# igormq/aes-lac-2018

Hardware: AMD Instinct MI355X
Metric: train frames/sec, DeepSpeech2 5xBiGRU-800 (higher is better)
Workload: dtype f32

## Files before the change

### aes-lac-2018_amd/csrc/bn.hip

```cpp
#include "ds2_common.h"

namespace {

constexpr int NPART = 64;

template <int MODE>
__global__ __launch_bounds__(256) void bn2d_reduce_kernel(const float* __restrict__ x, const float* __restrict__ dy,
                                                          const float* __restrict__ mean_invstd,
                                                          const float* __restrict__ gamma,
                                                          const float* __restrict__ beta, int B, int C, int inner,
                                                          double* __restrict__ part) {
    const int c = blockIdx.y, p = blockIdx.x, tid = threadIdx.x;
    const int chunks = (inner + 1023) / 1024;
    const int items = B * chunks;
    float mu = 0.f, is = 0.f, ga = 0.f, be = 0.f;
    if (MODE == 1) {
        mu = mean_invstd[c];
        is = mean_invstd[C + c];
        ga = gamma[c];
        be = beta[c];
    }
    float s0 = 0.f, s1 = 0.f;
    for (int it = p; it < items; it += NPART) {
        const int b = it / chunks, ch = it % chunks;
        const size_t base = ((size_t)b * C + c) * inner;
        const int i0 = ch * 1024;
#pragma unroll
        for (int u = 0; u < 4; ++u) {
            const int i = i0 + u * 256 + tid;
            if (i < inner) {
                const float v = x[base + i];
                if (MODE == 0) {
                    s0 += v;
                    s1 += v * v;
                } else {
                    const float xh = (v - mu) * is;
                    const float y = ga * xh + be;
                    const float g = (y > 0.f && y < 20.f) ? dy[base + i] : 0.f;
                    s0 += g;
                    s1 += g * xh;
                }
            }
        }
    }
    double d0 = wave_sum_d((double)s0), d1 = wave_sum_d((double)s1);
    __shared__ double sm[4][2];
    if ((tid & 63) == 0) {
        sm[tid >> 6][0] = d0;
        sm[tid >> 6][1] = d1;
    }
    __syncthreads();
    if (tid == 0) {
        part[((size_t)c * NPART + p) * 2 + 0] = sm[0][0] + sm[1][0] + sm[2][0] + sm[3][0];
        part[((size_t)c * NPART + p) * 2 + 1] = sm[0][1] + sm[1][1] + sm[2][1] + sm[3][1];
    }
}

template <int MODE>
__global__ __launch_bounds__(256) void bn2d_reduce_vec_kernel(const float* __restrict__ x, const float* __restrict__ dy,
                                                              const float* __restrict__ mean_invstd,
                                                              const float* __restrict__ gamma,
                                                              const float* __restrict__ beta, int B, int C, int inner,
                                                              double* __restrict__ part) {
    const int c = blockIdx.y, p = blockIdx.x, tid = threadIdx.x;
    const int chunks = (inner + 1023) / 1024;
    const int items = B * chunks;
    float mu = 0.f, is = 0.f, ga = 0.f, be = 0.f;
    if (MODE == 1) {
        mu = mean_invstd[c];
        is = mean_invstd[C + c];
        ga = gamma[c];
        be = beta[c];
    }
    float s0 = 0.f, s1 = 0.f;
    auto take = [&](float v, float g) {
        if (MODE == 0) {
            s0 += v;
            s1 += v * v;
        } else {
            const float xh = (v - mu) * is;
            const float y = ga * xh + be;
            const float gm = (y > 0.f && y < 20.f) ? g : 0.f;
            s0 += gm;
            s1 += gm * xh;
        }
    };
    for (int it = p; it < items; it += NPART) {
        const int b = it / chunks, ch = it % chunks;
        const size_t base = ((size_t)b * C + c) * inner;
        const int h = min((int)((4 - (base & 3)) & 3), inner);
        const int nq = (inner - h) >> 2;
        const int q = ch * 256 + tid;
        if (q < nq) {
            const f32x4 v = *reinterpret_cast<const f32x4*>(x + base + h + 4 * (size_t)q);
            f32x4 g = {0.f, 0.f, 0.f, 0.f};
            if (MODE == 1) g = *reinterpret_cast<const f32x4*>(dy + base + h + 4 * (size_t)q);
#pragma unroll
            for (int e = 0; e < 4; ++e) take(v[e], g[e]);
        }
        if (ch == 0) {
            const int tail0 = h + 4 * nq, e = tid < 4 ? tid : tail0 + tid - 4;
            if ((tid < h) || (tid >= 4 && tid < 8 && e < inner)) take(x[base + e], MODE == 1 ? dy[base + e] : 0.f);
        }
    }
    double d0 = wave_sum_d((double)s0), d1 = wave_sum_d((double)s1);
    __shared__ double sm[4][2];
    if ((tid & 63) == 0) {
        sm[tid >> 6][0] = d0;
        sm[tid >> 6][1] = d1;
    }
    __syncthreads();
    if (tid == 0) {
        part[((size_t)c * NPART + p) * 2 + 0] = sm[0][0] + sm[1][0] + sm[2][0] + sm[3][0];
        part[((size_t)c * NPART + p) * 2 + 1] = sm[0][1] + sm[1][1] + sm[2][1] + sm[3][1];
    }
}

template <int MODE>
__global__ __launch_bounds__(256) void bn1d_reduce_kernel(const float* __restrict__ xa, const float* __restrict__ xb,
                                                          const float* __restrict__ dy,
                                                          const float* __restrict__ mean_invstd, int rows, int F,
                                                          double* __restrict__ part) {
    const int p = blockIdx.x, tid = threadIdx.x;
    const int col = blockIdx.y * 64 + (tid & 63), ry = tid >> 6;
    float mu = 0.f, is = 0.f;
    if (MODE == 1 && col < F) {
        mu = mean_invstd[col];
        is = mean_invstd[F + col];
    }
    float s0 = 0.f, s1 = 0.f;
    if (col < F) {
        for (int r = p * 4 + ry; r < rows; r += NPART * 4) {
            const size_t o = (size_t)r * F + col;
            float v = xa[o];
            if (xb) v += xb[o];
            if (MODE == 0) {
                s0 += v;
                s1 += v * v;
            } else {
                const float g = dy[o];
                s0 += g;
                s1 += g * (v - mu) * is;
            }
        }
    }
    __shared__ float sm[4][64][2];
    sm[ry][tid & 63][0] = s0;
    sm[ry][tid & 63][1] = s1;
    __syncthreads();
    if (ry == 0 && col < F) {
        const int l = tid & 63;
        const double d0 = (double)sm[0][l][0] + (double)sm[1][l][0] + (double)sm[2][l][0] + (double)sm[3][l][0];
        const double d1 = (double)sm[0][l][1] + (double)sm[1][l][1] + (double)sm[2][l][1] + (double)sm[3][l][1];
        part[((size_t)col * NPART + p) * 2 + 0] = d0;
        part[((size_t)col * NPART + p) * 2 + 1] = d1;
    }
}

__global__ __launch_bounds__(64) void bn_finalize_stats_kernel(const double* __restrict__ part, int C, double count,
                                                               float eps, float momentum, int use_running,
                                                               float* __restrict__ running_mean,
                                                               float* __restrict__ running_var,
                                                               float* __restrict__ mean_invstd) {
    const int c = blockIdx.x, lane = threadIdx.x;
    if (use_running) {
        if (lane == 0) {
            mean_invstd[c] = running_mean[c];
            mean_invstd[C + c] = (float)(1.0 / sqrt((double)running_var[c] + (double)eps));
        }
        return;
    }
    double s0 = part[((size_t)c * NPART + lane) * 2 + 0];
    double s1 = part[((size_t)c * NPART + lane) * 2 + 1];
    s0 = wave_sum_d(s0);
    s1 = wave_sum_d(s1);
    if (lane == 0) {
        const double mean = s0 / count;
        double var = s1 / count - mean * mean;
        if (var < 0.0) var = 0.0;
        mean_invstd[c] = (float)mean;
        mean_invstd[C + c] = (float)(1.0 / sqrt(var + (double)eps));
        if (running_mean) {
            const double unb = count > 1.0 ? var * count / (count - 1.0) : var;
            running_mean[c] = (float)((1.0 - momentum) * running_mean[c] + momentum * mean);
            running_var[c] = (float)((1.0 - momentum) * running_var[c] + momentum * unb);
        }
    }
}

__global__ __launch_bounds__(64) void bn_finalize_bwd_kernel(const double* __restrict__ part, int C, double count,
                                                             float* __restrict__ dgamma, float* __restrict__ dbeta,
                                                             float* __restrict__ coef) {
    const int c = blockIdx.x, lane = threadIdx.x;
    double s0 = part[((size_t)c * NPART + lane) * 2 + 0];
    double s1 = part[((size_t)c * NPART + lane) * 2 + 1];
    s0 = wave_sum_d(s0);
    s1 = wave_sum_d(s1);
    if (lane == 0) {
        dbeta[c] = (float)s0;
        dgamma[c] = (float)s1;
        coef[c] = (float)(s0 / count);
        coef[C + c] = (float)(s1 / count);
    }
}

__global__ __launch_bounds__(256) void bn2d_apply_kernel(const float* __restrict__ x,
                                                         const float* __restrict__ mean_invstd,
                                                         const float* __restrict__ gamma,
                                                         const float* __restrict__ beta, int C, int inner,
                                                         float* __restrict__ y) {
    const int bc = blockIdx.y, c = bc % C;
    const float sc = gamma[c] * mean_invstd[C + c];
    const float sh = beta[c] - mean_invstd[c] * sc;
    const size_t base = (size_t)bc * inner;
    for (int i = blockIdx.x * 256 + threadIdx.x; i < inner; i += gridDim.x * 256) {
        const float v = x[base + i] * sc + sh;
        y[base + i] = fminf(fmaxf(v, 0.f), 20.f);
    }
}

__global__ __launch_bounds__(256) void bn2d_apply_tbf_kernel(const float* __restrict__ x,
                                                             const float* __restrict__ mean_invstd,
                                                             const float* __restrict__ gamma,
                                                             const float* __restrict__ beta, int B, int C, int D,
                                                             int T, float* __restrict__ y) {
    __shared__ float tile[32][33];
    const int b = blockIdx.z;
    const int CD = C * D;
    const int t0 = blockIdx.x * 32, f0 = blockIdx.y * 32;
    const int tx = threadIdx.x & 31, ty = threadIdx.x >> 5;
#pragma unroll
    for (int i = 0; i < 32; i += 8) {
        const int f = f0 + ty + i, t = t0 + tx;
        if (f < CD && t < T) {
            const int c = f / D;
            const float sc = gamma[c] * mean_invstd[C + c];
            const float sh = beta[c] - mean_invstd[c] * sc;
            const float v = x[((size_t)b * CD + f) * T + t] * sc + sh;
            tile[ty + i][tx] = fminf(fmaxf(v, 0.f), 20.f);
        }
    }
    __syncthreads();
#pragma unroll
    for (int i = 0; i < 32; i += 8) {
        const int t = t0 + ty + i, f = f0 + tx;
        if (f < CD && t < T) y[((size_t)t * B + b) * CD + f] = tile[tx][ty + i];
    }
}

__global__ __launch_bounds__(256) void bn2d_bwd_apply_kernel(const float* __restrict__ x, const float* __restrict__ dy,
                                                             const float* __restrict__ mean_invstd,
                                                             const float* __restrict__ gamma,
                                                             const float* __restrict__ beta,
                                                             const float* __restrict__ coef, int C, int inner,
                                                             float* __restrict__ dx) {
    const int bc = blockIdx.y, c = bc % C;
    const float mu = mean_invstd[c], is = mean_invstd[C + c], ga = gamma[c], be = beta[c];
    const float mg = coef[c], mgx = coef[C + c];
    const size_t base = (size_t)bc * inner;
    for (int i = blockIdx.x * 256 + threadIdx.x; i < inner; i += gridDim.x * 256) {
        const float xh = (x[base + i] - mu) * is;
        const float yv = ga * xh + be;
        const float g = (yv > 0.f && yv < 20.f) ? dy[base + i] : 0.f;
        dx[base + i] = ga * is * (g - mg - xh * mgx);
    }
}

template <typename F>
__device__ __forceinline__ void bn2d_row_vec(size_t base, int inner, F&& f4, int bx, int nbx, int tid) {
    const int h = min((int)((4 - (base & 3)) & 3), inner);
    const int nq = (inner - h) >> 2;
    for (int q = bx * 256 + tid; q < nq; q += nbx * 256) f4(base + h + 4 * (size_t)q, 4);
    if (bx == 0) {
        const int tail0 = h + 4 * nq, e = tid < 4 ? tid : tail0 + tid - 4;
        if ((tid < h) || (tid >= 4 && tid < 8 && e < inner)) f4(base + e, 1);
    }
}

__global__ __launch_bounds__(256) void bn2d_bwd_apply_vec_kernel(const float* __restrict__ x, const float* __restrict__ dy,
                                                                 const float* __restrict__ mean_invstd,
                                                                 const float* __restrict__ gamma,
                                                                 const float* __restrict__ beta,
                                                                 const float* __restrict__ coef, int C, int inner,
                                                                 float* __restrict__ dx) {
    const int bc = blockIdx.y, c = bc % C;
    const float mu = mean_invstd[c], is = mean_invstd[C + c], ga = gamma[c], be = beta[c];
    const float mg = coef[c], mgx = coef[C + c];
    auto one = [&](float xv, float g) {
        const float xh = (xv - mu) * is;
        const float yv = ga * xh + be;
        const float gm = (yv > 0.f && yv < 20.f) ? g : 0.f;
        return ga * is * (gm - mg - xh * mgx);
    };
    bn2d_row_vec((size_t)bc * inner, inner, [&](size_t o, int n) {
        if (n == 4) {
            const f32x4 xv = *reinterpret_cast<const f32x4*>(x + o), g = *reinterpret_cast<const f32x4*>(dy + o);
            f32x4 r;
#pragma unroll
            for (int e = 0; e < 4; ++e) r[e] = one(xv[e], g[e]);
            *reinterpret_cast<f32x4*>(dx + o) = r;
        } else {
            dx[o] = one(x[o], dy[o]);
        }
    }, blockIdx.x, gridDim.x, threadIdx.x);
}

__global__ __launch_bounds__(256) void bn2d_apply_vec_kernel(const float* __restrict__ x,
                                                             const float* __restrict__ mean_invstd,
                                                             const float* __restrict__ gamma,
                                                             const float* __restrict__ beta, int C, int inner,
                                                             float* __restrict__ y) {
    const int bc = blockIdx.y, c = bc % C;
    const float sc = gamma[c] * mean_invstd[C + c];
    const float sh = beta[c] - mean_invstd[c] * sc;
    bn2d_row_vec((size_t)bc * inner, inner, [&](size_t o, int n) {
        if (n == 4) {
            const f32x4 xv = *reinterpret_cast<const f32x4*>(x + o);
            f32x4 r;
#pragma unroll
            for (int e = 0; e < 4; ++e) r[e] = fminf(fmaxf(xv[e] * sc + sh, 0.f), 20.f);
            *reinterpret_cast<f32x4*>(y + o) = r;
        } else {
            y[o] = fminf(fmaxf(x[o] * sc + sh, 0.f), 20.f);
        }
    }, blockIdx.x, gridDim.x, threadIdx.x);
}

__global__ __launch_bounds__(256) void bn1d_apply_kernel(const float* __restrict__ xa, const float* __restrict__ xb,
                                                         const float* __restrict__ mean_invstd,
                                                         const float* __restrict__ gamma,
                                                         const float* __restrict__ beta, size_t n, int F,
                                                         float* __restrict__ y) {
    const size_t stride = (size_t)gridDim.x * 256;
    for (size_t i = (size_t)blockIdx.x * 256 + threadIdx.x; i < n; i += stride) {
        const int col = (int)(i % F);
        float v = xa[i];
        if (xb) v += xb[i];
        const float sc = gamma[col] * mean_invstd[F + col];
        y[i] = (v - mean_invstd[col]) * sc + beta[col];
    }
}

__global__ __launch_bounds__(256) void bn1d_bwd_apply_kernel(const float* __restrict__ xa, const float* __restrict__ xb,
                                                             const float* __restrict__ dy,
                                                             const float* __restrict__ mean_invstd,
                                                             const float* __restrict__ gamma,
                                                             const float* __restrict__ coef, size_t n, int F,
                                                             float* __restrict__ dx) {
    const size_t stride = (size_t)gridDim.x * 256;
    for (size_t i = (size_t)blockIdx.x * 256 + threadIdx.x; i < n; i += stride) {
        const int col = (int)(i % F);
        float v = xa[i];
        if (xb) v += xb[i];
        const float is = mean_invstd[F + col];
        const float xh = (v - mean_invstd[col]) * is;
        dx[i] = gamma[col] * is * (dy[i] - coef[col] - xh * coef[F + col]);
    }
}

template <int MODE>
__global__ __launch_bounds__(256) void bn1d_reduce_vec_kernel(const f32x4* __restrict__ xa, const f32x4* __restrict__ xb,
                                                              const f32x4* __restrict__ dy,
                                                              const float* __restrict__ mean_invstd, int rows, int F,
                                                              double* __restrict__ part) {
    const int p = blockIdx.x, tid = threadIdx.x;
    const int F4 = F >> 2;
    const int cq = blockIdx.y * 64 + (tid & 63), ry = tid >> 6;
    f32x4 mu = {0.f, 0.f, 0.f, 0.f}, is = mu;
    if (MODE == 1 && cq < F4) {
        mu = *reinterpret_cast<const f32x4*>(mean_invstd + 4 * cq);
        is = *reinterpret_cast<const f32x4*>(mean_invstd + F + 4 * cq);
    }
    f32x4 s0 = {0.f, 0.f, 0.f, 0.f}, s1 = s0;
    if (cq < F4) {
        for (int r = p * 4 + ry; r < rows; r += NPART * 4) {
            const size_t o = (size_t)r * F4 + cq;
            f32x4 v = xa[o];
            if (xb) v += xb[o];
            if (MODE == 0) {
                s0 += v;
                s1 += v * v;
            } else {
                const f32x4 g = dy[o];
                s0 += g;
                s1 += g * (v - mu) * is;
            }
        }
    }
    __shared__ f32x4 sm[4][64][2];
    sm[ry][tid & 63][0] = s0;
    sm[ry][tid & 63][1] = s1;
    __syncthreads();
    if (ry == 0 && cq < F4) {
        const int l = tid & 63;
#pragma unroll
        for (int e = 0; e < 4; ++e) {
            const double d0 = (double)sm[0][l][0][e] + (double)sm[1][l][0][e] + (double)sm[2][l][0][e] + (double)sm[3][l][0][e];
            const double d1 = (double)sm[0][l][1][e] + (double)sm[1][l][1][e] + (double)sm[2][l][1][e] + (double)sm[3][l][1][e];
            part[((size_t)(4 * cq + e) * NPART + p) * 2 + 0] = d0;
            part[((size_t)(4 * cq + e) * NPART + p) * 2 + 1] = d1;
        }
    }
}

__global__ __launch_bounds__(256) void bn1d_apply_vec_kernel(const f32x4* __restrict__ xa, const f32x4* __restrict__ xb,
                                                             const float* __restrict__ mean_invstd,
                                                             const float* __restrict__ gamma,
                                                             const float* __restrict__ beta, size_t n4, int F4,
                                                             f32x4* __restrict__ y) {
    const size_t stride = (size_t)gridDim.x * 256;
    for (size_t i = (size_t)blockIdx.x * 256 + threadIdx.x; i < n4; i += stride) {
        const int c = 4 * (int)(i % F4);
        f32x4 v = xa[i];
        if (xb) v += xb[i];
        const f32x4 sc = *reinterpret_cast<const f32x4*>(gamma + c) * *reinterpret_cast<const f32x4*>(mean_invstd + 4 * F4 + c);
        y[i] = (v - *reinterpret_cast<const f32x4*>(mean_invstd + c)) * sc + *reinterpret_cast<const f32x4*>(beta + c);
    }
}

__global__ __launch_bounds__(256) void bn1d_bwd_apply_vec_kernel(const f32x4* __restrict__ xa, const f32x4* __restrict__ xb,
                                                                 const f32x4* __restrict__ dy,
                                                                 const float* __restrict__ mean_invstd,
                                                                 const float* __restrict__ gamma,
                                                                 const float* __restrict__ coef, size_t n4, int F4,
                                                                 f32x4* __restrict__ dx) {
    const size_t stride = (size_t)gridDim.x * 256;
    const int F = 4 * F4;
    for (size_t i = (size_t)blockIdx.x * 256 + threadIdx.x; i < n4; i += stride) {
        const int c = 4 * (int)(i % F4);
        f32x4 v = xa[i];
        if (xb) v += xb[i];
        const f32x4 is = *reinterpret_cast<const f32x4*>(mean_invstd + F + c);
        const f32x4 xh = (v - *reinterpret_cast<const f32x4*>(mean_invstd + c)) * is;
        dx[i] = *reinterpret_cast<const f32x4*>(gamma + c) * is *
                (dy[i] - *reinterpret_cast<const f32x4*>(coef + c) - xh * *reinterpret_cast<const f32x4*>(coef + F + c));
    }
}

inline bool aligned16(const void* p) { return ((uintptr_t)p & 15) == 0; }
inline bool vec4_ok(int F, const void* a, const void* b, const void* c, const void* d) {
    return (F & 3) == 0 && ((((uintptr_t)a) | ((uintptr_t)b) | ((uintptr_t)c) | ((uintptr_t)d)) & 15) == 0;
}

inline int ew_blocks(size_t n) {
    size_t b = (n + 255) / 256;
    if (b > 4096) b = 4096;
    if (b < 1) b = 1;
    return (int)b;
}

}

extern "C" size_t ds2_bn_ws_bytes(int C) { return (size_t)C * NPART * 2 * sizeof(double) + (size_t)C * 2 * sizeof(float); }

extern "C" int ds2_bn2d_stats(const float* x, int B, int C, int inner, float eps, float momentum, int use_running,
                              float* running_mean, float* running_var, float* mean_invstd, void* ws, void* stream) {
    DS2_CHECK_ARG(x && mean_invstd && ws && B > 0 && C > 0 && inner > 0);
    DS2_CHECK_ARG(!use_running || (running_mean && running_var));
    DS2_CHECK_ARG((running_mean == nullptr) == (running_var == nullptr));
    DS2_CHECK_ARG(C <= 65535);
    hipStream_t st = (hipStream_t)stream;
    double* part = (double*)ws;
    if (!use_running) {
        if (aligned16(x))
            hipLaunchKernelGGL((bn2d_reduce_vec_kernel<0>), dim3(NPART, C), dim3(256), 0, st, x, nullptr, nullptr, nullptr,
                               nullptr, B, C, inner, part);
        else
            hipLaunchKernelGGL((bn2d_reduce_kernel<0>), dim3(NPART, C), dim3(256), 0, st, x, nullptr, nullptr, nullptr,
                               nullptr, B, C, inner, part);
    }
    hipLaunchKernelGGL(bn_finalize_stats_kernel, dim3(C), dim3(64), 0, st, part, C, (double)B * inner, eps, momentum,
                       use_running, running_mean, running_var, mean_invstd);
    DS2_CHECK_LAUNCH();
    return DS2_OK;
}

extern "C" int ds2_bn2d_apply_htanh(const float* x, const float* mean_invstd, const float* gamma, const float* beta,
                                    int B, int C, int D, int T, int layout_tbf, float* y, void* stream) {
    DS2_CHECK_ARG(x && mean_invstd && gamma && beta && y && B > 0 && C > 0 && D > 0 && T > 0);
    hipStream_t st = (hipStream_t)stream;
    if (layout_tbf) {
        DS2_CHECK_ARG(B <= 65535);
        dim3 grid(ds2_cdiv(T, 32), ds2_cdiv(C * D, 32), B);
        hipLaunchKernelGGL(bn2d_apply_tbf_kernel, grid, dim3(256), 0, st, x, mean_invstd, gamma, beta, B, C, D, T, y);
    } else {
        DS2_CHECK_ARG((long long)B * C <= 65535);
        const int inner = D * T;
        if (aligned16(x) && aligned16(y)) {
            dim3 grid(min(ds2_cdiv(inner, 1024), 64), B * C);
            hipLaunchKernelGGL(bn2d_apply_vec_kernel, grid, dim3(256), 0, st, x, mean_invstd, gamma, beta, C, inner, y);
        } else {
            dim3 grid(min(ds2_cdiv(inner, 256), 64), B * C);
            hipLaunchKernelGGL(bn2d_apply_kernel, grid, dim3(256), 0, st, x, mean_invstd, gamma, beta, C, inner, y);
        }
    }
    DS2_CHECK_LAUNCH();
    return DS2_OK;
}

extern "C" int ds2_bn2d_htanh_bwd(const float* x, const float* dy, const float* mean_invstd, const float* gamma,
                                  const float* beta, int B, int C, int D, int T, float* dx, float* dgamma,
                                  float* dbeta, void* ws, void* stream) {
    DS2_CHECK_ARG(x && dy && mean_invstd && gamma && beta && dx && dgamma && dbeta && ws);
    DS2_CHECK_ARG(B > 0 && C > 0 && D > 0 && T > 0);
    DS2_CHECK_ARG((long long)B * C <= 65535);
    hipStream_t st = (hipStream_t)stream;
    const int inner = D * T;
    double* part = (double*)ws;
    float* coef = (float*)(part + (size_t)C * NPART * 2);
    const bool vec = aligned16(x) && aligned16(dy) && aligned16(dx);
    if (vec)
        hipLaunchKernelGGL((bn2d_reduce_vec_kernel<1>), dim3(NPART, C), dim3(256), 0, st, x, dy, mean_invstd, gamma, beta,
                           B, C, inner, part);
    else
        hipLaunchKernelGGL((bn2d_reduce_kernel<1>), dim3(NPART, C), dim3(256), 0, st, x, dy, mean_invstd, gamma, beta, B,
                           C, inner, part);
    hipLaunchKernelGGL(bn_finalize_bwd_kernel, dim3(C), dim3(64), 0, st, part, C, (double)B * inner, dgamma, dbeta,
                       coef);
    if (vec) {
        dim3 grid(min(ds2_cdiv(inner, 1024), 64), B * C);
        hipLaunchKernelGGL(bn2d_bwd_apply_vec_kernel, grid, dim3(256), 0, st, x, dy, mean_invstd, gamma, beta, coef, C,
                           inner, dx);
    } else {
        dim3 grid(min(ds2_cdiv(inner, 256), 64), B * C);
        hipLaunchKernelGGL(bn2d_bwd_apply_kernel, grid, dim3(256), 0, st, x, dy, mean_invstd, gamma, beta, coef, C, inner,
                           dx);
    }
    DS2_CHECK_LAUNCH();
    return DS2_OK;
}

extern "C" int ds2_bn1d_stats(const float* xa, const float* xb, int rows, int F, float eps, float momentum,
                              int use_running, float* running_mean, float* running_var, float* mean_invstd, void* ws,
                              void* stream) {
    DS2_CHECK_ARG(xa && mean_invstd && ws && rows > 0 && F > 0);
    DS2_CHECK_ARG(!use_running || (running_mean && running_var));
    DS2_CHECK_ARG((running_mean == nullptr) == (running_var == nullptr));
    hipStream_t st = (hipStream_t)stream;
    double* part = (double*)ws;
    if (!use_running) {
        if (vec4_ok(F, xa, xb, nullptr, nullptr))
            hipLaunchKernelGGL((bn1d_reduce_vec_kernel<0>), dim3(NPART, ds2_cdiv(F / 4, 64)), dim3(256), 0, st,
                               (const f32x4*)xa, (const f32x4*)xb, nullptr, nullptr, rows, F, part);
        else
            hipLaunchKernelGGL((bn1d_reduce_kernel<0>), dim3(NPART, ds2_cdiv(F, 64)), dim3(256), 0, st, xa, xb, nullptr,
                               nullptr, rows, F, part);
    }
    hipLaunchKernelGGL(bn_finalize_stats_kernel, dim3(F), dim3(64), 0, st, part, F, (double)rows, eps, momentum,
                       use_running, running_mean, running_var, mean_invstd);
    DS2_CHECK_LAUNCH();
    return DS2_OK;
}

extern "C" int ds2_bn1d_apply(const float* xa, const float* xb, const float* mean_invstd, const float* gamma,
                              const float* beta, int rows, int F, float* y, void* stream) {
    DS2_CHECK_ARG(xa && mean_invstd && gamma && beta && y && rows > 0 && F > 0);
    const size_t n = (size_t)rows * F;
    if (vec4_ok(F, xa, xb, y, gamma) && vec4_ok(F, beta, mean_invstd, nullptr, nullptr))
        hipLaunchKernelGGL(bn1d_apply_vec_kernel, dim3(ew_blocks(n / 4)), dim3(256), 0, (hipStream_t)stream,
                           (const f32x4*)xa, (const f32x4*)xb, mean_invstd, gamma, beta, n / 4, F / 4, (f32x4*)y);
    else
        hipLaunchKernelGGL(bn1d_apply_kernel, dim3(ew_blocks(n)), dim3(256), 0, (hipStream_t)stream, xa, xb,
                           mean_invstd, gamma, beta, n, F, y);
    DS2_CHECK_LAUNCH();
    return DS2_OK;
}

extern "C" int ds2_bn1d_bwd(const float* xa, const float* xb, const float* dy, const float* mean_invstd,
                            const float* gamma, int rows, int F, float* dx, float* dgamma, float* dbeta, void* ws,
                            void* stream) {
    DS2_CHECK_ARG(xa && dy && mean_invstd && gamma && dx && dgamma && dbeta && ws && rows > 0 && F > 0);
    hipStream_t st = (hipStream_t)stream;
    double* part = (double*)ws;
    float* coef = (float*)(part + (size_t)F * NPART * 2);
    const bool vec = vec4_ok(F, xa, xb, dy, dx) && vec4_ok(F, gamma, mean_invstd, nullptr, nullptr);
    if (vec)
        hipLaunchKernelGGL((bn1d_reduce_vec_kernel<1>), dim3(NPART, ds2_cdiv(F / 4, 64)), dim3(256), 0, st,
                           (const f32x4*)xa, (const f32x4*)xb, (const f32x4*)dy, mean_invstd, rows, F, part);
    else
        hipLaunchKernelGGL((bn1d_reduce_kernel<1>), dim3(NPART, ds2_cdiv(F, 64)), dim3(256), 0, st, xa, xb, dy,
                           mean_invstd, rows, F, part);
    hipLaunchKernelGGL(bn_finalize_bwd_kernel, dim3(F), dim3(64), 0, st, part, F, (double)rows, dgamma, dbeta, coef);
    const size_t n = (size_t)rows * F;
    if (vec)
        hipLaunchKernelGGL(bn1d_bwd_apply_vec_kernel, dim3(ew_blocks(n / 4)), dim3(256), 0, st, (const f32x4*)xa,
                           (const f32x4*)xb, (const f32x4*)dy, mean_invstd, gamma, coef, n / 4, F / 4, (f32x4*)dx);
    else
        hipLaunchKernelGGL(bn1d_bwd_apply_kernel, dim3(ew_blocks(n)), dim3(256), 0, st, xa, xb, dy, mean_invstd, gamma,
                           coef, n, F, dx);
    DS2_CHECK_LAUNCH();
    return DS2_OK;
}
```

Baseline: 566,600.

## Fold BN statistic finalisation into reduce kernels via last-block arrival counters

Removes the separate finalize kernel launch for batch-norm stats and backward reductions: each reduce block publishes its partial and bumps a sharded per-stream atomic arrival counter, and the last arriving block combines partials and writes mean/invstd or dgamma/dbeta. The 1D partial layout is transposed to part-major so the combining block reads coalesced, and the 1D vectorised reduce is retiled to 16 column-quads by 16 rows with a 4-way unrolled load. The risks are relaxed-atomic memory-ordering correctness, plus the fixed slot table (limited streams and groups), which otherwise falls back to the old launch path.

Result: no change. 567,200 (median of 3 runs) (+0.1%).

```diff
diff --git a/aes-lac-2018_amd/csrc/bn.hip b/aes-lac-2018_amd/csrc/bn.hip
--- a/aes-lac-2018_amd/csrc/bn.hip
+++ b/aes-lac-2018_amd/csrc/bn.hip
@@ -1,15 +1,124 @@
+#include <mutex>
+
 #include "ds2_common.h"
 
 namespace {
 
 constexpr int NPART = 64;
+
+__device__ __forceinline__ void bn_write_stats(int c, int C, double s0, double s1, double count, float eps, float momentum,
+                                               float* __restrict__ running_mean, float* __restrict__ running_var,
+                                               float* __restrict__ mean_invstd) {
+    const double mean = s0 / count;
+    double var = s1 / count - mean * mean;
+    if (var < 0.0) var = 0.0;
+    mean_invstd[c] = (float)mean;
+    mean_invstd[C + c] = (float)(1.0 / sqrt(var + (double)eps));
+    if (running_mean) {
+        const double unb = count > 1.0 ? var * count / (count - 1.0) : var;
+        running_mean[c] = (float)((1.0 - momentum) * running_mean[c] + momentum * mean);
+        running_var[c] = (float)((1.0 - momentum) * running_var[c] + momentum * unb);
+    }
+}
+
+__device__ __forceinline__ void bn_write_bwd(int c, int C, double s0, double s1, double count, float* __restrict__ dgamma,
+                                             float* __restrict__ dbeta, float* __restrict__ coef) {
+    dbeta[c] = (float)s0;
+    dgamma[c] = (float)s1;
+    coef[c] = (float)(s0 / count);
+    coef[C + c] = (float)(s1 / count);
+}
+
+constexpr int BN_SLOTS = 8;
+constexpr int BN_GROUPS = 256;
+constexpr int BN_SHARDS = 8;
+struct BnArrivals {
+    unsigned int shard[BN_SHARDS][32];
+    unsigned int top[32];
+};
+__device__ BnArrivals g_bn_arrivals[BN_SLOTS][BN_GROUPS];
+
+struct BnFold {
+    int slot, C;
+    double count;
+    float eps, momentum;
+    float *running_mean, *running_var, *mean_invstd;
+    float *dgamma, *dbeta, *coef;
+};
+
+__device__ __forceinline__ void put_partial(double* p, double v) {
+    __hip_atomic_store(p, v, __ATOMIC_RELAXED, __HIP_MEMORY_SCOPE_AGENT);
+}
+
+template <int MODE, bool SEQ>
+__device__ __forceinline__ void bn_combine(const double* part, const BnFold& f, int c0, int nc) {
+    auto write = [&](int c, double t0, double t1) {
+        if (MODE == 0)
+            bn_write_stats(c, f.C, t0, t1, f.count, f.eps, f.momentum, f.running_mean, f.running_var, f.mean_invstd);
+        else
+            bn_write_bwd(c, f.C, t0, t1, f.count, f.dgamma, f.dbeta, f.coef);
+    };
+    const int q = threadIdx.x >> 6, j = threadIdx.x & 63;
+    if (!SEQ) {
+        for (int c = c0 + q; c < c0 + nc; c += 4) {
+            const double* p = part + ((size_t)c * NPART + j) * 2;
+            const double t0 = wave_sum_d(__hip_atomic_load(p, __ATOMIC_RELAXED, __HIP_MEMORY_SCOPE_AGENT));
+            const double t1 = wave_sum_d(__hip_atomic_load(p + 1, __ATOMIC_RELAXED, __HIP_MEMORY_SCOPE_AGENT));
+            if (j == 0) write(c, t0, t1);
+        }
+        return;
+    }
+    __shared__ double s_quarter[4][64][2];
+    double s0 = 0.0, s1 = 0.0;
+    if (j < nc) {
+        double v0[16], v1[16];
+#pragma unroll
+        for (int i = 0; i < 16; ++i) {
+            const double* p = part + ((size_t)(16 * q + i) * f.C + c0 + j) * 2;
+            v0[i] = __hip_atomic_load(p, __ATOMIC_RELAXED, __HIP_MEMORY_SCOPE_AGENT);
+            v1[i] = __hip_atomic_load(p + 1, __ATOMIC_RELAXED, __HIP_MEMORY_SCOPE_AGENT);
+        }
+#pragma unroll
+        for (int i = 0; i < 16; ++i) {
+            s0 += v0[i];
+            s1 += v1[i];
+        }
+    }
+    s_quarter[q][j][0] = s0;
+    s_quarter[q][j][1] = s1;
+    __syncthreads();
+    if (q == 0 && j < nc)
+        write(c0 + j, ((s_quarter[0][j][0] + s_quarter[1][j][0]) + s_quarter[2][j][0]) + s_quarter[3][j][0],
+              ((s_quarter[0][j][1] + s_quarter[1][j][1]) + s_quarter[2][j][1]) + s_quarter[3][j][1]);
+}
+
+template <int MODE, bool SEQ>
+__device__ __forceinline__ void bn_fold(const double* part, const BnFold& f, int group, int c0, int nc) {
+    if (f.slot < 0) return;
+    __shared__ int s_last;
+    __builtin_amdgcn_s_waitcnt(0x0F70);
+    __syncthreads();
+    if (threadIdx.x == 0) {
+        BnArrivals& a = g_bn_arrivals[f.slot][group];
+        unsigned int* shard = &a.shard[blockIdx.x % BN_SHARDS][0];
+        bool last = false;
+        if (__hip_atomic_fetch_add(shard, 1u, __ATOMIC_RELAXED, __HIP_MEMORY_SCOPE_AGENT) == (unsigned)(NPART / BN_SHARDS - 1)) {
+            __hip_atomic_store(shard, 0u, __ATOMIC_RELAXED, __HIP_MEMORY_SCOPE_AGENT);
+            last = __hip_atomic_fetch_add(&a.top[0], 1u, __ATOMIC_RELAXED, __HIP_MEMORY_SCOPE_AGENT) == (unsigned)(BN_SHARDS - 1);
+            if (last) __hip_atomic_store(&a.top[0], 0u, __ATOMIC_RELAXED, __HIP_MEMORY_SCOPE_AGENT);
+        }
+        s_last = last;
+    }
+    __syncthreads();
+    if (s_last) bn_combine<MODE, SEQ>(part, f, c0, nc);
+}
 
 template <int MODE>
 __global__ __launch_bounds__(256) void bn2d_reduce_kernel(const float* __restrict__ x, const float* __restrict__ dy,
                                                           const float* __restrict__ mean_invstd,
                                                           const float* __restrict__ gamma,
                                                           const float* __restrict__ beta, int B, int C, int inner,
-                                                          double* __restrict__ part) {
+                                                          double* __restrict__ part, BnFold fold) {
     const int c = blockIdx.y, p = blockIdx.x, tid = threadIdx.x;
     const int chunks = (inner + 1023) / 1024;
     const int items = B * chunks;
@@ -51,9 +160,10 @@
     }
     __syncthreads();
     if (tid == 0) {
-        part[((size_t)c * NPART + p) * 2 + 0] = sm[0][0] + sm[1][0] + sm[2][0] + sm[3][0];
-        part[((size_t)c * NPART + p) * 2 + 1] = sm[0][1] + sm[1][1] + sm[2][1] + sm[3][1];
-    }
+        put_partial(part + ((size_t)c * NPART + p) * 2 + 0, sm[0][0] + sm[1][0] + sm[2][0] + sm[3][0]);
+        put_partial(part + ((size_t)c * NPART + p) * 2 + 1, sm[0][1] + sm[1][1] + sm[2][1] + sm[3][1]);
+    }
+    bn_fold<MODE, false>(part, fold, c, c, 1);
 }
 
 template <int MODE>
@@ -61,7 +171,7 @@
                                                               const float* __restrict__ mean_invstd,
                                                               const float* __restrict__ gamma,
                                                               const float* __restrict__ beta, int B, int C, int inner,
-                                                              double* __restrict__ part) {
+                                                              double* __restrict__ part, BnFold fold) {
     const int c = blockIdx.y, p = blockIdx.x, tid = threadIdx.x;
     const int chunks = (inner + 1023) / 1024;
     const int items = B * chunks;
@@ -111,16 +221,17 @@
     }
     __syncthreads();
     if (tid == 0) {
-        part[((size_t)c * NPART + p) * 2 + 0] = sm[0][0] + sm[1][0] + sm[2][0] + sm[3][0];
-        part[((size_t)c * NPART + p) * 2 + 1] = sm[0][1] + sm[1][1] + sm[2][1] + sm[3][1];
-    }
+        put_partial(part + ((size_t)c * NPART + p) * 2 + 0, sm[0][0] + sm[1][0] + sm[2][0] + sm[3][0]);
+        put_partial(part + ((size_t)c * NPART + p) * 2 + 1, sm[0][1] + sm[1][1] + sm[2][1] + sm[3][1]);
+    }
+    bn_fold<MODE, false>(part, fold, c, c, 1);
 }
 
 template <int MODE>
 __global__ __launch_bounds__(256) void bn1d_reduce_kernel(const float* __restrict__ xa, const float* __restrict__ xb,
                                                           const float* __restrict__ dy,
                                                           const float* __restrict__ mean_invstd, int rows, int F,
-                                                          double* __restrict__ part) {
+                                                          double* __restrict__ part, BnFold fold) {
     const int p = blockIdx.x, tid = threadIdx.x;
     const int col = blockIdx.y * 64 + (tid & 63), ry = tid >> 6;
     float mu = 0.f, is = 0.f;
@@ -152,56 +263,31 @@
         const int l = tid & 63;
         const double d0 = (double)sm[0][l][0] + (double)sm[1][l][0] + (double)sm[2][l][0] + (double)sm[3][l][0];
         const double d1 = (double)sm[0][l][1] + (double)sm[1][l][1] + (double)sm[2][l][1] + (double)sm[3][l][1];
-        part[((size_t)col * NPART + p) * 2 + 0] = d0;
-        part[((size_t)col * NPART + p) * 2 + 1] = d1;
-    }
-}
-
-__global__ __launch_bounds__(64) void bn_finalize_stats_kernel(const double* __restrict__ part, int C, double count,
-                                                               float eps, float momentum, int use_running,
-                                                               float* __restrict__ running_mean,
-                                                               float* __restrict__ running_var,
-                                                               float* __restrict__ mean_invstd) {
-    const int c = blockIdx.x, lane = threadIdx.x;
+        put_partial(part + ((size_t)p * F + col) * 2 + 0, d0);
+        put_partial(part + ((size_t)p * F + col) * 2 + 1, d1);
+    }
+    bn_fold<MODE, true>(part, fold, blockIdx.y, blockIdx.y * 64, min(64, F - (int)blockIdx.y * 64));
+}
+
+constexpr int bn_fin(bool seq) { return seq ? 64 : 4; }
+template <bool SEQ>
+__global__ __launch_bounds__(256) void bn_finalize_stats_kernel(const double* __restrict__ part, BnFold f, int use_running) {
+    const int c0 = blockIdx.x * bn_fin(SEQ);
     if (use_running) {
-        if (lane == 0) {
-            mean_invstd[c] = running_mean[c];
-            mean_invstd[C + c] = (float)(1.0 / sqrt((double)running_var[c] + (double)eps));
+        const int c = c0 + threadIdx.x;
+        if (threadIdx.x < bn_fin(SEQ) && c < f.C) {
+            f.mean_invstd[c] = f.running_mean[c];
+            f.mean_invstd[f.C + c] = (float)(1.0 / sqrt((double)f.running_var[c] + (double)f.eps));
         }
         return;
     }
-    double s0 = part[((size_t)c * NPART + lane) * 2 + 0];
-    double s1 = part[((size_t)c * NPART + lane) * 2 + 1];
-    s0 = wave_sum_d(s0);
-    s1 = wave_sum_d(s1);
-    if (lane == 0) {
-        const double mean = s0 / count;
-        double var = s1 / count - mean * mean;
-        if (var < 0.0) var = 0.0;
-        mean_invstd[c] = (float)mean;
-        mean_invstd[C + c] = (float)(1.0 / sqrt(var + (double)eps));
-        if (running_mean) {
-            const double unb = count > 1.0 ? var * count / (count - 1.0) : var;
-            running_mean[c] = (float)((1.0 - momentum) * running_mean[c] + momentum * mean);
-            running_var[c] = (float)((1.0 - momentum) * running_var[c] + momentum * unb);
-        }
-    }
-}
-
-__global__ __launch_bounds__(64) void bn_finalize_bwd_kernel(const double* __restrict__ part, int C, double count,
-                                                             float* __restrict__ dgamma, float* __restrict__ dbeta,
-                                                             float* __restrict__ coef) {
-    const int c = blockIdx.x, lane = threadIdx.x;
-    double s0 = part[((size_t)c * NPART + lane) * 2 + 0];
-    double s1 = part[((size_t)c * NPART + lane) * 2 + 1];
-    s0 = wave_sum_d(s0);
-    s1 = wave_sum_d(s1);
-    if (lane == 0) {
-        dbeta[c] = (float)s0;
-        dgamma[c] = (float)s1;
-        coef[c] = (float)(s0 / count);
-        coef[C + c] = (float)(s1 / count);
-    }
+    bn_combine<0, SEQ>(part, f, c0, min(bn_fin(SEQ), f.C - c0));
+}
+
+template <bool SEQ>
+__global__ __launch_bounds__(256) void bn_finalize_bwd_kernel(const double* __restrict__ part, BnFold f) {
+    const int c0 = blockIdx.x * bn_fin(SEQ);
+    bn_combine<1, SEQ>(part, f, c0, min(bn_fin(SEQ), f.C - c0));
 }
 
 __global__ __launch_bounds__(256) void bn2d_apply_kernel(const float* __restrict__ x,
@@ -362,10 +448,11 @@
 __global__ __launch_bounds__(256) void bn1d_reduce_vec_kernel(const f32x4* __restrict__ xa, const f32x4* __restrict__ xb,
                                                               const f32x4* __restrict__ dy,
                                                               const float* __restrict__ mean_invstd, int rows, int F,
-                                                              double* __restrict__ part) {
+                                                              double* __restrict__ part, BnFold fold) {
     const int p = blockIdx.x, tid = threadIdx.x;
     const int F4 = F >> 2;
-    const int cq = blockIdx.y * 64 + (tid & 63), ry = tid >> 6;
+    const int lq = tid & 15, ry = tid >> 4;
+    const int cq = blockIdx.y * 16 + lq;
     f32x4 mu = {0.f, 0.f, 0.f, 0.f}, is = mu;
     if (MODE == 1 && cq < F4) {
         mu = *reinterpret_cast<const f32x4*>(mean_invstd + 4 * cq);
@@ -373,34 +460,44 @@
     }
     f32x4 s0 = {0.f, 0.f, 0.f, 0.f}, s1 = s0;
     if (cq < F4) {
-        for (int r = p * 4 + ry; r < rows; r += NPART * 4) {
-            const size_t o = (size_t)r * F4 + cq;
-            f32x4 v = xa[o];
-            if (xb) v += xb[o];
-            if (MODE == 0) {
-                s0 += v;
-                s1 += v * v;
-            } else {
-                const f32x4 g = dy[o];
-                s0 += g;
-                s1 += g * (v - mu) * is;
+        for (int r0 = p * 16 + ry; r0 < rows; r0 += 4 * NPART * 16) {
+            f32x4 v[4], g[4];
+#pragma unroll
+            for (int u = 0; u < 4; ++u) {
+                const int r = r0 + u * NPART * 16;
+                if (r < rows) {
+                    const size_t o = (size_t)r * F4 + cq;
+                    v[u] = xa[o];
+                    if (xb) v[u] += xb[o];
+                    if (MODE == 1) g[u] = dy[o];
+                }
             }
-        }
-    }
-    __shared__ f32x4 sm[4][64][2];
-    sm[ry][tid & 63][0] = s0;
-    sm[ry][tid & 63][1] = s1;
+#pragma unroll
+            for (int u = 0; u < 4; ++u) {
+                if (r0 + u * NPART * 16 < rows) {
+                    if (MODE == 0) {
+                        s0 += v[u];
+                        s1 += v[u] * v[u];
+                    } else {
+                        s0 += g[u];
+                        s1 += g[u] * (v[u] - mu) * is;
+                    }
+                }
+            }
+        }
+    }
+    __shared__ f32x4 sm[16][16][2];
+    sm[ry][lq][0] = s0;
+    sm[ry][lq][1] = s1;
     __syncthreads();
-    if (ry == 0 && cq < F4) {
-        const int l = tid & 63;
-#pragma unroll
-        for (int e = 0; e < 4; ++e) {
-            const double d0 = (double)sm[0][l][0][e] + (double)sm[1][l][0][e] + (double)sm[2][l][0][e] + (double)sm[3][l][0][e];
-            const double d1 = (double)sm[0][l][1][e] + (double)sm[1][l][1][e] + (double)sm[2][l][1][e] + (double)sm[3][l][1][e];
-            part[((size_t)(4 * cq + e) * NPART + p) * 2 + 0] = d0;
-            part[((size_t)(4 * cq + e) * NPART + p) * 2 + 1] = d1;
-        }
-    }
+    const int j = tid >> 1, s = tid & 1, col = blockIdx.y * 64 + j;
+    if (tid < 128 && col < F) {
+        double d = 0.0;
+#pragma unroll
+        for (int y = 0; y < 16; ++y) d += (double)reinterpret_cast<const float*>(&sm[y][j >> 2][s])[j & 3];
+        put_partial(part + ((size_t)p * F + col) * 2 + s, d);
+    }
+    bn_fold<MODE, true>(part, fold, blockIdx.y, blockIdx.y * 64, min(64, F - (int)blockIdx.y * 64));
 }
 
 __global__ __launch_bounds__(256) void bn1d_apply_vec_kernel(const f32x4* __restrict__ xa, const f32x4* __restrict__ xb,
@@ -449,6 +546,29 @@
     return (int)b;
 }
 
+int bn_slot(hipStream_t st, int groups) {
+    static std::mutex mu;
+    static hipStream_t owner[BN_SLOTS];
+    static int taken = 0;
+    if (groups > BN_GROUPS) return -1;
+    std::lock_guard<std::mutex> lock(mu);
+    for (int i = 0; i < taken; ++i)
+        if (owner[i] == st) return i;
+    if (taken == BN_SLOTS) return -1;
+    owner[taken] = st;
+    return taken++;
+}
+
+BnFold fold_stats(int slot, int C, double count, float eps, float momentum, float* running_mean, float* running_var,
+                  float* mean_invstd) {
+    return BnFold{slot, C, count, eps, momentum, running_mean, running_var, mean_invstd,
+                  nullptr, nullptr, nullptr};
+}
+
+BnFold fold_bwd(int slot, int C, double count, float* dgamma, float* dbeta, float* coef) {
+    return BnFold{slot, C, count, 0.f, 0.f, nullptr, nullptr, nullptr, dgamma, dbeta, coef};
+}
+
 }
 
 extern "C" size_t ds2_bn_ws_bytes(int C) { return (size_t)C * NPART * 2 * sizeof(double) + (size_t)C * 2 * sizeof(float); }
@@ -461,16 +581,19 @@
     DS2_CHECK_ARG(C <= 65535);
     hipStream_t st = (hipStream_t)stream;
     double* part = (double*)ws;
+    BnFold fold = fold_stats(use_running ? -1 : bn_slot(st, C), C, (double)B * inner, eps, momentum, running_mean,
+                             running_var, mean_invstd);
     if (!use_running) {
         if (aligned16(x))
             hipLaunchKernelGGL((bn2d_reduce_vec_kernel<0>), dim3(NPART, C), dim3(256), 0, st, x, nullptr, nullptr, nullptr,
-                               nullptr, B, C, inner, part);
+                               nullptr, B, C, inner, part, fold);
         else
             hipLaunchKernelGGL((bn2d_reduce_kernel<0>), dim3(NPART, C), dim3(256), 0, st, x, nullptr, nullptr, nullptr,
-                               nullptr, B, C, inner, part);
-    }
-    hipLaunchKernelGGL(bn_finalize_stats_kernel, dim3(C), dim3(64), 0, st, part, C, (double)B * inner, eps, momentum,
-                       use_running, running_mean, running_var, mean_invstd);
+                               nullptr, B, C, inner, part, fold);
+    }
+    if (fold.slot < 0)
+        hipLaunchKernelGGL(bn_finalize_stats_kernel<false>, dim3(ds2_cdiv(C, bn_fin(false))), dim3(256), 0, st, part, fold,
+                           use_running);
     DS2_CHECK_LAUNCH();
     return DS2_OK;
 }
@@ -509,14 +632,15 @@
     double* part = (double*)ws;
     float* coef = (float*)(part + (size_t)C * NPART * 2);
     const bool vec = aligned16(x) && aligned16(dy) && aligned16(dx);
+    const BnFold fold = fold_bwd(bn_slot(st, C), C, (double)B * inner, dgamma, dbeta, coef);
     if (vec)
         hipLaunchKernelGGL((bn2d_reduce_vec_kernel<1>), dim3(NPART, C), dim3(256), 0, st, x, dy, mean_invstd, gamma, beta,
-                           B, C, inner, part);
+                           B, C, inner, part, fold);
     else
         hipLaunchKernelGGL((bn2d_reduce_kernel<1>), dim3(NPART, C), dim3(256), 0, st, x, dy, mean_invstd, gamma, beta, B,
-                           C, inner, part);
-    hipLaunchKernelGGL(bn_finalize_bwd_kernel, dim3(C), dim3(64), 0, st, part, C, (double)B * inner, dgamma, dbeta,
-                       coef);
+                           C, inner, part, fold);
+    if (fold.slot < 0)
+        hipLaunchKernelGGL(bn_finalize_bwd_kernel<false>, dim3(ds2_cdiv(C, bn_fin(false))), dim3(256), 0, st, part, fold);
     if (vec) {
         dim3 grid(min(ds2_cdiv(inner, 1024), 64), B * C);
         hipLaunchKernelGGL(bn2d_bwd_apply_vec_kernel, grid, dim3(256), 0, st, x, dy, mean_invstd, gamma, beta, coef, C,
@@ -538,16 +662,19 @@
     DS2_CHECK_ARG((running_mean == nullptr) == (running_var == nullptr));
     hipStream_t st = (hipStream_t)stream;
     double* part = (double*)ws;
+    const BnFold fold = fold_stats(use_running ? -1 : bn_slot(st, ds2_cdiv(F, 64)), F, (double)rows, eps, momentum,
+                                   running_mean, running_var, mean_invstd);
     if (!use_running) {
         if (vec4_ok(F, xa, xb, nullptr, nullptr))
-            hipLaunchKernelGGL((bn1d_reduce_vec_kernel<0>), dim3(NPART, ds2_cdiv(F / 4, 64)), dim3(256), 0, st,
-                               (const f32x4*)xa, (const f32x4*)xb, nullptr, nullptr, rows, F, part);
+            hipLaunchKernelGGL((bn1d_reduce_vec_kernel<0>), dim3(NPART, ds2_cdiv(F / 4, 16)), dim3(256), 0, st,
+                               (const f32x4*)xa, (const f32x4*)xb, nullptr, nullptr, rows, F, part, fold);
         else
             hipLaunchKernelGGL((bn1d_reduce_kernel<0>), dim3(NPART, ds2_cdiv(F, 64)), dim3(256), 0, st, xa, xb, nullptr,
-                               nullptr, rows, F, part);
-    }
-    hipLaunchKernelGGL(bn_finalize_stats_kernel, dim3(F), dim3(64), 0, st, part, F, (double)rows, eps, momentum,
-                       use_running, running_mean, running_var, mean_invstd);
+                               nullptr, rows, F, part, fold);
+    }
+    if (fold.slot < 0)
+        hipLaunchKernelGGL(bn_finalize_stats_kernel<true>, dim3(ds2_cdiv(F, bn_fin(true))), dim3(256), 0, st, part, fold,
+                           use_running);
     DS2_CHECK_LAUNCH();
     return DS2_OK;
 }
@@ -574,13 +701,15 @@
     double* part = (double*)ws;
     float* coef = (float*)(part + (size_t)F * NPART * 2);
     const bool vec = vec4_ok(F, xa, xb, dy, dx) && vec4_ok(F, gamma, mean_invstd, nullptr, nullptr);
+    const BnFold fold = fold_bwd(bn_slot(st, ds2_cdiv(F, 64)), F, (double)rows, dgamma, dbeta, coef);
     if (vec)
-        hipLaunchKernelGGL((bn1d_reduce_vec_kernel<1>), dim3(NPART, ds2_cdiv(F / 4, 64)), dim3(256), 0, st,
-                           (const f32x4*)xa, (const f32x4*)xb, (const f32x4*)dy, mean_invstd, rows, F, part);
+        hipLaunchKernelGGL((bn1d_reduce_vec_kernel<1>), dim3(NPART, ds2_cdiv(F / 4, 16)), dim3(256), 0, st,
+                           (const f32x4*)xa, (const f32x4*)xb, (const f32x4*)dy, mean_invstd, rows, F, part, fold);
     else
         hipLaunchKernelGGL((bn1d_reduce_kernel<1>), dim3(NPART, ds2_cdiv(F, 64)), dim3(256), 0, st, xa, xb, dy,
-                           mean_invstd, rows, F, part);
-    hipLaunchKernelGGL(bn_finalize_bwd_kernel, dim3(F), dim3(64), 0, st, part, F, (double)rows, dgamma, dbeta, coef);
+                           mean_invstd, rows, F, part, fold);
+    if (fold.slot < 0)
+        hipLaunchKernelGGL(bn_finalize_bwd_kernel<true>, dim3(ds2_cdiv(F, bn_fin(true))), dim3(256), 0, st, part, fold);
     const size_t n = (size_t)rows * F;
     if (vec)
         hipLaunchKernelGGL(bn1d_bwd_apply_vec_kernel, dim3(ew_blocks(n / 4)), dim3(256), 0, st, (const f32x4*)xa,
```
